# Y-Claw/Multilevel-GNN

Measured on AMD Instinct MI355X. Metric: graphs/sec fwd+bwd, 3-level GNN on 10k-node d=128 synthetic; HBM GB/s %peak, higher is better.
Workload: dtype f32; 1 GPU; configs[1]: ER graphs N=10000 E=160000 x64 per GPU, d=128, 3 GENConv(softmax, res+, LayerNorm) + projection pooling G=25000 k=2 + DiffPool 146->37->10, fp32; step = CSR build (of the next batch, on a second stream) + fwd + bwd + grad all-reduce + Adam; graphs_per_gpu=64, global_batch=64, parallelism=dp1, world_size=1, allreduce_bytes=1429768

## Files before the change

### multilevel-gnn_amd/csrc/densesage.hip

```cpp
#include "common.h"
#include "launch.h"
#include "mlgnn.h"
#include "tile_gemm.h"

namespace mlgnn {

constexpr int kDsMaxN = 160, kDsMaxC = 128, kDsMaxO = 64, kDsMaxNAdj = 48;
constexpr int kDsBlock = 1024, kDsWaves = kDsBlock / kWave;
constexpr float kDsNormEps = 1e-12f;
constexpr int kDsFwdTiles = 3;
static_assert(kDsFwdTiles * (kDsWaves / (kDsMaxO / 16)) >= kDsMaxN / 16, "row tiles of one column tile per wave");

struct DsArgs {
  const void* x; const void* adj; const void* w_rel; const void* w_root; const float* bias;
  const void* gy; const void* y; const float* rinv_in;
  void* y_out; float* rinv; void* gx; void* gadj; float* ws;
  int n; int C; int O; int adj_batched; int normalize; int ws_cols;
  int vec16;
};

template <typename AB>
__device__ __forceinline__ void ds_degrees(const AB ab, int n, int stride, float* deg, float* raw) {
  const int lane = threadIdx.x & (kWave - 1), wave = threadIdx.x / kWave;
  for (int r = wave; r < n; r += kDsWaves) {
    float s = 0.f;
    for (int j = lane; j < n; j += kWave) s += ab[(size_t)r * stride + j];
#pragma unroll
    for (int off = 32; off > 0; off >>= 1) s += __shfl_xor(s, off);
    if (lane == 0) {
      if (raw) raw[r] = s;
      deg[r] = fmaxf(s, 1.0f);
    }
  }
}

struct DsLds { int so, sx, sa, np, op; };
__host__ __device__ inline DsLds ds_lds(int n, int C, int O) {
  DsLds l;
  l.np = (n + 15) & ~15;
  l.op = (O + 15) & ~15;
  l.so = l.op + 1;
  l.sx = ((C + 31) & ~31) + 1;
  l.sa = ((n + 31) & ~31) + 1;
  return l;
}
__host__ __device__ inline int ds_fwd_floats(const DsLds& l) {
  const int first = l.np * l.sx + 2 * l.op * l.sx, then = l.np * (l.sx > l.sa ? l.sx : l.sa) + l.np * l.so;
  return first > then ? first : then;
}
inline size_t ds_fwd_lds_bytes(int n, int C, int O) {
  const DsLds l = ds_lds(n, C, O);
  return ((size_t)ds_fwd_floats(l) + l.np) * 4;
}
inline size_t ds_bwd_lds_bytes(int n, int C, int O, bool adj_grad) {
  const DsLds l = ds_lds(n, C, O);
  size_t f = (size_t)2 * l.np * l.so + 2 * l.np;
  if (adj_grad) f += (size_t)l.np * l.so + (size_t)l.np * (l.np + 1);
  return f * 4;
}

template <typename T, int V>
__device__ __forceinline__ void ds_stage_run(float* img, int stride, const T* src, int cols, int first, int count) {
  const int step = V * kDsBlock, dr = step / cols, dc = step - dr * cols;
  int e = first + V * (int)threadIdx.x;
  int r = e / cols, c = e - r * cols;
  for (int i = threadIdx.x; i < count; i += kDsBlock, e += step) {
    float v[V];
    load_t<T, V>(v, src + e);
    int rr = r, cc = c;
#pragma unroll
    for (int q = 0; q < V; ++q) {
      img[rr * stride + cc] = v[q];
      if (++cc == cols) { cc = 0; ++rr; }
    }
    c += dc; r += dr;
    if (c >= cols) { c -= cols; ++r; }
  }
}

template <typename T>
__device__ __forceinline__ void ds_stage(float* img, int stride, const T* src, int rows, int cols, int rows_p,
                                         int cols_p, int vec16) {
  constexpr int V = 16 / (int)sizeof(T);
  const int lane = threadIdx.x & (kWave - 1), wave = threadIdx.x / kWave;
  const int total = rows * cols;
  int head = total;
  if (vec16) head = min(total, (int)(((0 - reinterpret_cast<uintptr_t>(src)) & 15) / sizeof(T)));
  const int nvec = (total - head) / V;
  ds_stage_run<T, 1>(img, stride, src, cols, 0, head);
  if (nvec > 0) ds_stage_run<T, V>(img, stride, src, cols, head, nvec);
  ds_stage_run<T, 1>(img, stride, src, cols, head + V * nvec, total - head - V * nvec);
  for (int r = wave; r < rows_p; r += kDsWaves)
    for (int c = (r < rows ? cols : 0) + lane; c < cols_p; c += kWave) img[r * stride + c] = 0.f;
}

template <typename T>
__global__ __launch_bounds__(kDsBlock) void dense_sage_fwd_kernel(const DsArgs p) {
  extern __shared__ __attribute__((aligned(16))) float ds_smem[];
  const int b = blockIdx.x, tid = threadIdx.x;
  const int lane = tid & (kWave - 1), wave = tid / kWave;
  const int n = p.n, C = p.C, O = p.O;
  const DsLds L = ds_lds(n, C, O);
  const int SO = L.so, SX = L.sx, SA = L.sa;
  float* Xm_ = ds_smem;
  float* Wr_ = Xm_ + (size_t)L.np * SX;
  float* Wt_ = Wr_ + (size_t)L.op * SX;
  float* Am_ = Xm_;
  float* deg = ds_smem + ds_fwd_floats(L);
  float* Pm_ = deg - (size_t)L.np * SO;
#define P(r, c) Pm_[(r) * SO + (c)]
#define X(r, c) Xm_[(r) * SX + (c)]
#define A(r, c) Am_[(r) * SA + (c)]
  const T* xg = static_cast<const T*>(p.x) + (size_t)b * n * C;
  const T* ag = static_cast<const T*>(p.adj) + (p.adj_batched ? (size_t)b * n * n : 0);
  const int NP = (n + 15) & ~15, OP = (O + 15) & ~15;
  const int Nt = NP / 16, Ot = OP / 16;
  const int l15 = lane & 15, lq = lane >> 4;
  const int wpc = kDsWaves / Ot, j0 = (wave % Ot) * 16, first = wave / Ot;
  const bool active = first < wpc;

  ds_stage<T>(Xm_, SX, xg, n, C, NP, SX - 1, p.vec16);
  ds_stage<T>(Wr_, SX, static_cast<const T*>(p.w_rel), O, C, OP, SX - 1, p.vec16);
  ds_stage<T>(Wt_, SX, static_cast<const T*>(p.w_root), O, C, OP, SX - 1, p.vec16);
  __syncthreads();
  f32x4 keep[kDsFwdTiles];
  for_k_blocks<kDsMaxC / 32>((C + 31) >> 5, [&](auto kb) {
    constexpr int KB = decltype(kb)::value;
    float wr[8 * KB], wt[8 * KB];
    if (active) {
      frag_load<KB>(wr, [&](int k) { return Wr_[(j0 + l15) * SX + k]; });
      frag_load<KB>(wt, [&](int k) { return Wt_[(j0 + l15) * SX + k]; });
    }
    __syncthreads();
    if (active) {
#pragma unroll
      for (int s = 0; s < kDsFwdTiles; ++s) {
        const int i0 = (first + s * wpc) * 16;
        if (i0 < NP) {
          f32x4 acc;
          tile_gemm2_b_resident<KB>(wr, wt, [&](int i, int k) { return X(i0 + i, k); }, acc, keep[s]);
#pragma unroll
          for (int r = 0; r < 4; ++r) P(i0 + lq * 4 + r, j0 + l15) = acc[r];
        }
      }
    }
  });
  __syncthreads();
  ds_stage<T>(Am_, SA, ag, n, n, NP, (n + 31) & ~31, p.vec16);
  __syncthreads();
  ds_degrees(Am_, n, SA, deg, nullptr);
  f32x4 agg[kDsFwdTiles];
  if (active) {
#pragma unroll
    for (int s = 0; s < kDsFwdTiles; ++s) {
      const int i0 = (first + s * wpc) * 16;
      if (i0 < NP)
        agg[s] = tile_gemm(n,
            [&](int i, int k) { return A(i0 + i, k); },
            [&](int k, int j) { return k < n ? P(k, j0 + j) : 0.f; });
    }
  }
  __syncthreads();
  if (active) {
    const float bj = (p.bias && j0 + l15 < O) ? p.bias[j0 + l15] : 0.f;
#pragma unroll
    for (int s = 0; s < kDsFwdTiles; ++s) {
      const int i0 = (first + s * wpc) * 16;
      if (i0 < NP) {
#pragma unroll
        for (int r = 0; r < 4; ++r) {
          const int row = i0 + lq * 4 + r;
          P(row, j0 + l15) = agg[s][r] / deg[min(row, n - 1)] + keep[s][r] + bj;
        }
      }
    }
  }
  __syncthreads();
  for (int r = wave; r < n; r += kDsWaves) {
    const float v = lane < O ? P(r, lane) : 0.f;
    float ss = v * v;
#pragma unroll
    for (int off = 32; off > 0; off >>= 1) ss += __shfl_xor(ss, off);
    const float ri = p.normalize ? 1.0f / fmaxf(sqrtf(ss), kDsNormEps) : 1.0f;
    if (lane < O) stored_write<T>(p.y_out, ((size_t)b * n + r) * O + lane, v * ri);
    if (lane == 0) p.rinv[(size_t)b * n + r] = ri;
  }
}
#undef P
#undef X
#undef A

template <typename T>
__global__ __launch_bounds__(kDsBlock) void dense_sage_bwd_kernel(const DsArgs p) {
  extern __shared__ __attribute__((aligned(16))) float ds_smem[];
  const int b = blockIdx.x, tid = threadIdx.x;
  const int lane = tid & (kWave - 1), wave = tid / kWave;
  const int n = p.n, C = p.C, O = p.O;
  const DsLds L = ds_lds(n, C, O);
  const int SO = L.so, SM = L.np + 1;
  float* G_ = ds_smem;
  float* GP_ = G_ + (size_t)L.np * SO;
  float* deg = GP_ + (size_t)L.np * SO;
  float* raw = deg + L.np;
  float* Pm_ = raw + L.np;
  float* M_ = Pm_ + (size_t)L.np * SO;
#define G(r, c) G_[(r) * SO + (c)]
#define GP(r, c) GP_[(r) * SO + (c)]
#define Pm(r, c) Pm_[(r) * SO + (c)]
#define M(r, c) M_[(r) * SM + (c)]
  const StoredIn<T> xb{static_cast<const T*>(p.x) + (size_t)b * n * C};
  const StoredIn<T> ab{static_cast<const T*>(p.adj) + (p.adj_batched ? (size_t)b * n * n : 0)};
  const StoredIn<T> w_rel{static_cast<const T*>(p.w_rel)}, w_root{static_cast<const T*>(p.w_root)};
  const StoredIn<T> gyb{static_cast<const T*>(p.gy) + (size_t)b * n * O};
  const StoredIn<T> yb{static_cast<const T*>(p.y) + (size_t)b * n * O};
  const int NP = (n + 15) & ~15, OP = (O + 15) & ~15, CP = (C + 15) & ~15;
  const int Nt = NP / 16, Ot = OP / 16, Ct = CP / 16;
  const int l15 = lane & 15, lq = lane >> 4;

  ds_degrees(ab, n, n, deg, raw);
  for (int r = wave; r < NP; r += kDsWaves) {
    float gv = 0.f, yv = 0.f;
    if (r < n && lane < O) { gv = gyb[(size_t)r * O + lane]; yv = yb[(size_t)r * O + lane]; }
    float dot = gv * yv;
#pragma unroll
    for (int off = 32; off > 0; off >>= 1) dot += __shfl_xor(dot, off);
    const float ri = r < n ? p.rinv_in[(size_t)b * n + r] : 0.f;
    const float g = p.normalize ? (gv - yv * dot) * ri : gv;
    if (lane < OP) G(r, lane) = (r < n && lane < O) ? g : 0.f;
  }
  __syncthreads();
  for (int t = wave; t < Nt * Ot; t += kDsWaves) {
    const int i0 = (t / Ot) * 16, j0 = (t % Ot) * 16;
    const f32x4 acc = tile_gemm(n,
        [&](int i, int k) { return (i0 + i < n && k < n) ? ab[(size_t)k * n + i0 + i] : 0.f; },
        [&](int k, int j) { return k < n ? G(k, j0 + j) / deg[k] : 0.f; });
#pragma unroll
    for (int r = 0; r < 4; ++r) GP(i0 + lq * 4 + r, j0 + l15) = acc[r];
  }
  __syncthreads();
  const size_t gx_off = (size_t)b * n * C;
  for (int t = wave; t < Nt * Ct; t += kDsWaves) {
    const int i0 = (t / Ct) * 16, c0 = (t % Ct) * 16;
    f32x4 acc = tile_gemm(O,
        [&](int i, int k) { return k < O ? GP(i0 + i, k) : 0.f; },
        [&](int k, int j) { return (k < O && c0 + j < C) ? w_rel[(size_t)k * C + c0 + j] : 0.f; });
    const f32x4 t2 = tile_gemm(O,
        [&](int i, int k) { return k < O ? G(i0 + i, k) : 0.f; },
        [&](int k, int j) { return (k < O && c0 + j < C) ? w_root[(size_t)k * C + c0 + j] : 0.f; });
#pragma unroll
    for (int r = 0; r < 4; ++r) {
      const int row = i0 + lq * 4 + r, col = c0 + l15;
      if (row < n && col < C) stored_write<T>(p.gx, gx_off + (size_t)row * C + col, acc[r] + t2[r]);
    }
  }
  float* wsb = p.ws + (size_t)b * p.ws_cols;
  for (int t = wave; t < 2 * Ot * Ct; t += kDsWaves) {
    const int which = t / (Ot * Ct), tt = t % (Ot * Ct);
    const int o0 = (tt / Ct) * 16, c0 = (tt % Ct) * 16;
    const float* src = which == 0 ? GP_ : G_;
    const f32x4 acc = tile_gemm(n,
        [&](int i, int k) { return k < n ? src[k * SO + o0 + i] : 0.f; },
        [&](int k, int j) { return (k < n && c0 + j < C) ? xb[(size_t)k * C + c0 + j] : 0.f; });
#pragma unroll
    for (int r = 0; r < 4; ++r) {
      const int o = o0 + lq * 4 + r, c = c0 + l15;
      if (o < O && c < C) wsb[(size_t)which * O * C + (size_t)o * C + c] = acc[r];
    }
  }
  for (int o = tid; o < O; o += kDsBlock) {
    float s = 0.f;
    for (int r = 0; r < n; ++r) s += G(r, o);
    wsb[(size_t)2 * O * C + o] = s;
  }
  if (p.gadj) {
    for (int t = wave; t < Nt * Ot; t += kDsWaves) {
      const int i0 = (t / Ot) * 16, j0 = (t % Ot) * 16;
      const f32x4 acc = tile_gemm(C,
          [&](int i, int k) { return (i0 + i < n && k < C) ? xb[(size_t)(i0 + i) * C + k] : 0.f; },
          [&](int k, int j) { return (j0 + j < O && k < C) ? w_rel[(size_t)(j0 + j) * C + k] : 0.f; });
#pragma unroll
      for (int r = 0; r < 4; ++r) Pm(i0 + lq * 4 + r, j0 + l15) = acc[r];
    }
    __syncthreads();
    for (int t = wave; t < Nt * Nt; t += kDsWaves) {
      const int i0 = (t / Nt) * 16, j0 = (t % Nt) * 16;
      const f32x4 acc = tile_gemm(O,
          [&](int i, int k) { return k < O ? G(i0 + i, k) : 0.f; },
          [&](int k, int j) { return k < O ? Pm(j0 + j, k) : 0.f; });
#pragma unroll
      for (int r = 0; r < 4; ++r) M(i0 + lq * 4 + r, j0 + l15) = acc[r];
    }
    __syncthreads();
    const size_t ga_off = (size_t)b * n * n;
    for (int r = wave; r < n; r += kDsWaves) {
      float c = lane < n ? ab[(size_t)r * n + lane] * M(r, lane) : 0.f;
#pragma unroll
      for (int off = 32; off > 0; off >>= 1) c += __shfl_xor(c, off);
      const float ci = raw[r] >= 1.0f ? c / deg[r] : 0.f;
      if (lane < n) stored_write<T>(p.gadj, ga_off + (size_t)r * n + lane, (M(r, lane) - ci) / deg[r]);
    }
  }
}
#undef G
#undef GP
#undef Pm
#undef M

static bool ds_dims_ok(int64_t n, int64_t C, int64_t O) {
  return n >= 1 && n <= kDsMaxN && C >= 1 && C <= kDsMaxC && O >= 1 && O <= kDsMaxO;
}

}

using namespace mlgnn;

extern "C" int mlgnn_dense_sage_supported(int64_t n, int64_t C, int64_t O, int need_grad_adj) {
  return (ds_dims_ok(n, C, O) && (!need_grad_adj || n <= kDsMaxNAdj)) ? 1 : 0;
}

extern "C" int64_t mlgnn_dense_sage_bwd_workspace_floats(int64_t B, int64_t C, int64_t O) {
  if (B < 0 || C <= 0 || O <= 0) return MLGNN_E_SHAPE;
  return B * (2 * O * C + O);
}

extern "C" int mlgnn_dense_sage_fwd(const void* x, const void* adj, const void* w_rel, const void* w_root,
                                    const float* bias, void* y, float* rinv, int64_t B, int64_t n, int64_t C,
                                    int64_t O, int adj_batched, int normalize, int dtype, void* stream) {
  if (dtype != MLGNN_DTYPE_F32 && dtype != MLGNN_DTYPE_BF16) return MLGNN_E_DTYPE;
  if (B < 0 || !ds_dims_ok(n, C, O)) return MLGNN_E_SHAPE;
  if (B == 0) return 0;
  if (!x || !adj || !w_rel || !w_root || !y || !rinv) return MLGNN_E_NULL;
  DsArgs a = {};
  a.x = x; a.adj = adj; a.w_rel = w_rel; a.w_root = w_root;
  a.bias = bias; a.y_out = y; a.rinv = rinv;
  a.n = (int)n; a.C = (int)C; a.O = (int)O; a.adj_batched = adj_batched; a.normalize = normalize;
  a.vec16 = aligned<16>(x, adj, w_rel, w_root) ? 1 : 0;
  const size_t lds = ds_fwd_lds_bytes((int)n, (int)C, (int)O);
  static size_t fwd_attr = 0;
  if (lds > fwd_attr) {
    const int most = (int)ds_fwd_lds_bytes(kDsMaxN, kDsMaxC, kDsMaxO);
    if (const hipError_t e = allow_dynamic_lds(&dense_sage_fwd_kernel<float>, most); e != hipSuccess) return (int)e;
    if (const hipError_t e = allow_dynamic_lds(&dense_sage_fwd_kernel<bf16_t>, most); e != hipSuccess) return (int)e;
    fwd_attr = (size_t)most;
  }
  if (dtype == MLGNN_DTYPE_BF16) hipLaunchKernelGGL(dense_sage_fwd_kernel<bf16_t>, dim3((unsigned)B), dim3(kDsBlock), lds, (hipStream_t)stream, a);
  else hipLaunchKernelGGL(dense_sage_fwd_kernel<float>, dim3((unsigned)B), dim3(kDsBlock), lds, (hipStream_t)stream, a);
  return (int)hipGetLastError();
}

extern "C" int mlgnn_dense_sage_bwd(const void* grad_y, const void* y, const float* rinv, const void* x,
                                    const void* adj, const void* w_rel, const void* w_root, void* grad_x,
                                    void* grad_adj, float* grad_w, float* workspace, int64_t workspace_floats,
                                    int64_t B, int64_t n, int64_t C, int64_t O, int adj_batched, int normalize,
                                    int dtype, void* stream) {
  if (dtype != MLGNN_DTYPE_F32 && dtype != MLGNN_DTYPE_BF16) return MLGNN_E_DTYPE;
  if (B < 0 || !ds_dims_ok(n, C, O)) return MLGNN_E_SHAPE;
  if (grad_adj && n > kDsMaxNAdj) return MLGNN_E_SHAPE;
  if (!grad_w) return MLGNN_E_NULL;
  const int cols = (int)(2 * O * C + O);
  hipStream_t s = (hipStream_t)stream;
  if (B == 0) return (int)hipMemsetAsync(grad_w, 0, (size_t)cols * 4, s);
  if (!grad_y || !y || !rinv || !x || !adj || !w_rel || !w_root || !grad_x || !workspace) return MLGNN_E_NULL;
  if (workspace_floats < B * cols) return MLGNN_E_WORKSPACE;
  DsArgs a = {};
  a.x = x; a.adj = adj; a.w_rel = w_rel; a.w_root = w_root;
  a.gy = grad_y; a.y = y; a.rinv_in = rinv;
  a.gx = grad_x; a.gadj = grad_adj; a.ws = workspace; a.ws_cols = cols;
  a.n = (int)n; a.C = (int)C; a.O = (int)O; a.adj_batched = adj_batched; a.normalize = normalize;
  const size_t lds = ds_bwd_lds_bytes((int)n, (int)C, (int)O, grad_adj != nullptr);
  static size_t bwd_attr = 0;
  if (lds > bwd_attr) {
    const size_t most = ds_bwd_lds_bytes(kDsMaxN, kDsMaxC, kDsMaxO, false) > ds_bwd_lds_bytes(kDsMaxNAdj, kDsMaxC, kDsMaxO, true)
                            ? ds_bwd_lds_bytes(kDsMaxN, kDsMaxC, kDsMaxO, false) : ds_bwd_lds_bytes(kDsMaxNAdj, kDsMaxC, kDsMaxO, true);
    if (const hipError_t e = allow_dynamic_lds(&dense_sage_bwd_kernel<float>, (int)most); e != hipSuccess) return (int)e;
    if (const hipError_t e = allow_dynamic_lds(&dense_sage_bwd_kernel<bf16_t>, (int)most); e != hipSuccess) return (int)e;
    bwd_attr = most;
  }
  if (dtype == MLGNN_DTYPE_BF16) hipLaunchKernelGGL(dense_sage_bwd_kernel<bf16_t>, dim3((unsigned)B), dim3(kDsBlock), lds, s, a);
  else hipLaunchKernelGGL(dense_sage_bwd_kernel<float>, dim3((unsigned)B), dim3(kDsBlock), lds, s, a);
  int err = (int)hipGetLastError();
  if (err) return err;
  launch_reduce_partials(workspace, grad_w, (int)B, cols, s);
  return (int)hipGetLastError();
}
```

### multilevel-gnn_amd/csrc/tile_gemm.h

```cpp
#pragma once
#include "split_precision.h"
#include "dispatch.h"

namespace mlgnn {

constexpr int kTileUnroll = 8;

template <typename FA, typename FB>
__device__ __forceinline__ f32x4 tile_gemm(int kdim, FA a_at, FB b_at) {
  const int lane = threadIdx.x & (kWave - 1);
  const int l15 = lane & 15, lk = lane >> 4;
  f32x4 acc = {0.f, 0.f, 0.f, 0.f};
  for (int k0 = 0; k0 < kdim; k0 += 4 * kTileUnroll) {
    float a[kTileUnroll], b[kTileUnroll];
#pragma unroll
    for (int u = 0; u < kTileUnroll; ++u) {
      a[u] = a_at(l15, k0 + 4 * u + lk);
      b[u] = b_at(k0 + 4 * u + lk, l15);
    }
#pragma unroll
    for (int u = 0; u < kTileUnroll; ++u) acc = __builtin_amdgcn_mfma_f32_16x16x4f32(a[u], b[u], acc, 0, 0, 0);
  }
  return acc;
}

template <int KB, typename F>
__device__ __forceinline__ void frag_load(float (&f)[8 * KB], F at) {
  const int lk = (threadIdx.x & (kWave - 1)) >> 4;
#pragma unroll
  for (int u = 0; u < 8 * KB; ++u) f[u] = at(4 * u + lk);
}

template <int KB, typename FA>
__device__ __forceinline__ void tile_gemm2_b_resident(const float (&b0)[8 * KB], const float (&b1)[8 * KB], FA a_at,
                                                      f32x4& acc0, f32x4& acc1) {
  const int lane = threadIdx.x & (kWave - 1);
  const int l15 = lane & 15, lk = lane >> 4;
  acc0 = f32x4{0.f, 0.f, 0.f, 0.f};
  acc1 = f32x4{0.f, 0.f, 0.f, 0.f};
#pragma unroll
  for (int blk = 0; blk < KB; ++blk) {
    float a[kTileUnroll];
#pragma unroll
    for (int u = 0; u < kTileUnroll; ++u) a[u] = a_at(l15, 32 * blk + 4 * u + lk);
#pragma unroll
    for (int u = 0; u < kTileUnroll; ++u) {
      acc0 = __builtin_amdgcn_mfma_f32_16x16x4f32(a[u], b0[8 * blk + u], acc0, 0, 0, 0);
      acc1 = __builtin_amdgcn_mfma_f32_16x16x4f32(a[u], b1[8 * blk + u], acc1, 0, 0, 0);
    }
  }
}

template <int MAXKB, typename F>
__device__ __forceinline__ void for_k_blocks(int kb, F&& f) {
  if constexpr (MAXKB > 1) {
    if (kb < MAXKB) { for_k_blocks<MAXKB - 1>(kb, f); return; }
  }
  f(IC<MAXKB>{});
}

}
```

Measured before the change: 5557 graphs/s.

## Stage adjacency, weights and features in LDS for dense SAGE backward

The DiffPool dense SAGE backward kernel can now copy the adjacency, both weight matrices and the node features into shared memory whenever they fit and there are enough tiles to reuse them. All GEMMs then read from LDS instead of re-reading global memory per tile. Alongside that, it prefetches gy/y/rinv into registers so those loads overlap the adjacency staging, and folds the 1/deg scaling into the degree pass. It also keeps weight fragments in registers across row tiles for the gx GEMM and unrolls the bias-gradient sum. The cost is added LDS footprint near the 160 KiB limit, extra barriers, and an env var that forces either path.

```diff
diff --git a/multilevel-gnn_amd/csrc/densesage.hip b/multilevel-gnn_amd/csrc/densesage.hip
--- a/multilevel-gnn_amd/csrc/densesage.hip
+++ b/multilevel-gnn_amd/csrc/densesage.hip
@@ -1,3 +1,5 @@
+#include <cstdlib>
+
 #include "common.h"
 #include "launch.h"
 #include "mlgnn.h"
@@ -9,6 +11,9 @@
 constexpr int kDsBlock = 1024, kDsWaves = kDsBlock / kWave;
 constexpr float kDsNormEps = 1e-12f;
 constexpr int kDsFwdTiles = 3;
+constexpr int kDsRows = kDsMaxN / kDsWaves;
+static_assert(kDsRows * kDsWaves == kDsMaxN, "every padded row of g has a wave");
+constexpr int kDsGpTiles = ((kDsMaxN / 16) * (kDsMaxO / 16) + kDsWaves - 1) / kDsWaves;
 static_assert(kDsFwdTiles * (kDsWaves / (kDsMaxO / 16)) >= kDsMaxN / 16, "row tiles of one column tile per wave");
 
 struct DsArgs {
@@ -31,6 +36,19 @@
       if (raw) raw[r] = s;
       deg[r] = fmaxf(s, 1.0f);
     }
+  }
+}
+
+template <typename AB, typename F>
+__device__ __forceinline__ void ds_degrees_each(const AB ab, int n, int stride, float* deg, float* raw, F each) {
+  const int lane = threadIdx.x & (kWave - 1), wave = threadIdx.x / kWave;
+  for (int r = wave; r < n; r += kDsWaves) {
+    float s = 0.f;
+    for (int j = lane; j < n; j += kWave) s += ab[(size_t)r * stride + j];
+#pragma unroll
+    for (int off = 32; off > 0; off >>= 1) s += __shfl_xor(s, off);
+    if (lane == 0) { raw[r] = s; deg[r] = fmaxf(s, 1.0f); }
+    each(r, fmaxf(s, 1.0f));
   }
 }
 
@@ -52,11 +70,44 @@
   const DsLds l = ds_lds(n, C, O);
   return ((size_t)ds_fwd_floats(l) + l.np) * 4;
 }
-inline size_t ds_bwd_lds_bytes(int n, int C, int O, bool adj_grad) {
-  const DsLds l = ds_lds(n, C, O);
-  size_t f = (size_t)2 * l.np * l.so + 2 * l.np;
-  if (adj_grad) f += (size_t)l.np * l.so + (size_t)l.np * (l.np + 1);
-  return f * 4;
+constexpr int kDsLdsBytes = 160 * 1024;
+struct DsBwdLds { int np, so, sa, sw, base, xo, floats; };
+__host__ __device__ constexpr DsBwdLds ds_bwd_lds(int n, int C, int O, bool adj_grad, bool images) {
+  DsBwdLds l = {};
+  l.np = (n + 15) & ~15;
+  l.so = ((O + 15) & ~15) + 1;
+  l.sa = ((n + 31) & ~31) + 1;
+  l.sw = ((C + 31) & ~31) + (adj_grad ? 17 : 16);
+  l.base = 2 * l.np * l.so + 2 * l.np + (adj_grad ? l.np * l.so + l.np * (l.np + 1) : 0);
+  const int a = n * l.sa, w = 2 * O * l.sw, x = n * l.sw;
+  l.xo = adj_grad ? w : 0;
+  const int wx = adj_grad ? w + x : (w > x ? w : x);
+  l.floats = l.base + (images ? (a > wx ? a : wx) : 0);
+  return l;
+}
+constexpr size_t ds_bwd_lds_bytes(int n, int C, int O, bool adj_grad, bool images) {
+  return (size_t)ds_bwd_lds(n, C, O, adj_grad, images).floats * 4;
+}
+constexpr bool ds_bwd_images_fit(int n, int C, int O, bool adj_grad) {
+  return ds_bwd_lds_bytes(n, C, O, adj_grad, true) <= (size_t)kDsLdsBytes;
+}
+constexpr bool ds_bwd_images_pay(int n, int C, int O) {
+  const int nt = (n + 15) / 16, ct = (C + 15) / 16, ot = (O + 15) / 16;
+  return nt * ot + nt * ct + 2 * ot * ct > kDsWaves;
+}
+static_assert(ds_bwd_images_fit(146, 128, 37, false) && ds_bwd_images_fit(146, 128, 32, false), "level 1");
+static_assert(ds_bwd_images_pay(146, 128, 37) && ds_bwd_images_pay(146, 128, 32), "level 1");
+static_assert(ds_bwd_lds_bytes(146, 128, 37, false, true) == 158024, "level 1: n rows of the adjacency, not 160");
+static_assert(ds_bwd_images_fit(37, 32, 32, true) && ds_bwd_images_fit(37, 32, 10, true) &&
+              ds_bwd_images_fit(37, 32, 64, true) && ds_bwd_images_fit(10, 64, 64, true), "levels 2 and 3");
+static_assert(ds_bwd_images_pay(37, 32, 32) && ds_bwd_images_pay(37, 32, 64) && ds_bwd_images_pay(10, 64, 64) &&
+              !ds_bwd_images_pay(37, 32, 10), "levels 2 and 3: the 10-channel assignment conv keeps global operands");
+static_assert(ds_bwd_images_fit(146, 128, 48, false) && !ds_bwd_images_fit(146, 128, 49, false), "O <= 48 at n = 146");
+static_assert(ds_bwd_images_fit(kDsMaxNAdj, kDsMaxC, kDsMaxO, true), "every shape with the adjacency gradient");
+static_assert(!ds_bwd_images_fit(kDsMaxN, kDsMaxC, kDsMaxO, false), "x + g + gP alone exceed the LDS there");
+inline int ds_bwd_path_forced() {
+  static const int v = [] { const char* e = getenv("MLGNN_DS_BWD_GLOBAL"); return !e ? -1 : e[0] == '1' ? 1 : e[0] == '0' ? 0 : -1; }();
+  return v;
 }
 
 template <typename T, int V>
@@ -190,26 +241,31 @@
 #undef X
 #undef A
 
-template <typename T>
+template <typename T, bool IMG>
 __global__ __launch_bounds__(kDsBlock) void dense_sage_bwd_kernel(const DsArgs p) {
   extern __shared__ __attribute__((aligned(16))) float ds_smem[];
   const int b = blockIdx.x, tid = threadIdx.x;
   const int lane = tid & (kWave - 1), wave = tid / kWave;
   const int n = p.n, C = p.C, O = p.O;
-  const DsLds L = ds_lds(n, C, O);
-  const int SO = L.so, SM = L.np + 1;
+  const DsBwdLds L = ds_bwd_lds(n, C, O, p.gadj != nullptr, IMG);
+  const int SO = L.so, SM = L.np + 1, SA = L.sa, SW = L.sw;
   float* G_ = ds_smem;
   float* GP_ = G_ + (size_t)L.np * SO;
   float* deg = GP_ + (size_t)L.np * SO;
   float* raw = deg + L.np;
   float* Pm_ = raw + L.np;
   float* M_ = Pm_ + (size_t)L.np * SO;
+  float* Am_ = ds_smem + L.base;
+  float* Wr_ = Am_;
+  float* Wt_ = Wr_ + (size_t)O * SW;
+  float* Xm_ = Am_ + L.xo;
 #define G(r, c) G_[(r) * SO + (c)]
 #define GP(r, c) GP_[(r) * SO + (c)]
 #define Pm(r, c) Pm_[(r) * SO + (c)]
 #define M(r, c) M_[(r) * SM + (c)]
-  const StoredIn<T> xb{static_cast<const T*>(p.x) + (size_t)b * n * C};
-  const StoredIn<T> ab{static_cast<const T*>(p.adj) + (p.adj_batched ? (size_t)b * n * n : 0)};
+  const T* xg = static_cast<const T*>(p.x) + (size_t)b * n * C;
+  const T* ag = static_cast<const T*>(p.adj) + (p.adj_batched ? (size_t)b * n * n : 0);
+  const StoredIn<T> xb{xg}, ab{ag};
   const StoredIn<T> w_rel{static_cast<const T*>(p.w_rel)}, w_root{static_cast<const T*>(p.w_root)};
   const StoredIn<T> gyb{static_cast<const T*>(p.gy) + (size_t)b * n * O};
   const StoredIn<T> yb{static_cast<const T*>(p.y) + (size_t)b * n * O};
@@ -217,42 +273,95 @@
   const int Nt = NP / 16, Ot = OP / 16, Ct = CP / 16;
   const int l15 = lane & 15, lq = lane >> 4;
 
-  ds_degrees(ab, n, n, deg, raw);
-  for (int r = wave; r < NP; r += kDsWaves) {
-    float gv = 0.f, yv = 0.f;
-    if (r < n && lane < O) { gv = gyb[(size_t)r * O + lane]; yv = yb[(size_t)r * O + lane]; }
-    float dot = gv * yv;
-#pragma unroll
-    for (int off = 32; off > 0; off >>= 1) dot += __shfl_xor(dot, off);
-    const float ri = r < n ? p.rinv_in[(size_t)b * n + r] : 0.f;
-    const float g = p.normalize ? (gv - yv * dot) * ri : gv;
-    if (lane < OP) G(r, lane) = (r < n && lane < O) ? g : 0.f;
-  }
-  __syncthreads();
-  for (int t = wave; t < Nt * Ot; t += kDsWaves) {
-    const int i0 = (t / Ot) * 16, j0 = (t % Ot) * 16;
-    const f32x4 acc = tile_gemm(n,
-        [&](int i, int k) { return (i0 + i < n && k < n) ? ab[(size_t)k * n + i0 + i] : 0.f; },
-        [&](int k, int j) { return k < n ? G(k, j0 + j) / deg[k] : 0.f; });
-#pragma unroll
-    for (int r = 0; r < 4; ++r) GP(i0 + lq * 4 + r, j0 + l15) = acc[r];
-  }
-  __syncthreads();
+  float gv[kDsRows], yv[kDsRows], ri[kDsRows];
+#pragma unroll
+  for (int s = 0; s < kDsRows; ++s) {
+    const int r = wave + s * kDsWaves;
+    gv[s] = yv[s] = ri[s] = 0.f;
+    if (r < n) {
+      if (lane < O) { gv[s] = gyb[(size_t)r * O + lane]; yv[s] = yb[(size_t)r * O + lane]; }
+      ri[s] = p.rinv_in[(size_t)b * n + r];
+    }
+  }
+  if constexpr (IMG) ds_stage<T>(Am_, SA, ag, n, n, n, n, p.vec16);
+#pragma unroll
+  for (int s = 0; s < kDsRows; ++s) {
+    const int r = wave + s * kDsWaves;
+    if (r < NP) {
+      float dot = gv[s] * yv[s];
+#pragma unroll
+      for (int off = 32; off > 0; off >>= 1) dot += __shfl_xor(dot, off);
+      const float g = p.normalize ? (gv[s] - yv[s] * dot) * ri[s] : gv[s];
+      if (lane < OP) G(r, lane) = (r < n && lane < O) ? g : 0.f;
+    }
+  }
+  if constexpr (IMG) __syncthreads();
+  const auto scale_row = [&](int r, float d) { if (lane < OP) GP(r, lane) = G(r, lane) / d; };
+  if constexpr (IMG) ds_degrees_each(Am_, n, SA, deg, raw, scale_row);
+  else ds_degrees_each(ab, n, n, deg, raw, scale_row);
+  __syncthreads();
+  f32x4 gp[kDsGpTiles];
+#pragma unroll
+  for (int s = 0; s < kDsGpTiles; ++s) {
+    const int t = wave + s * kDsWaves;
+    if (t < Nt * Ot) {
+      const int i0 = (t / Ot) * 16, j0 = (t % Ot) * 16;
+      gp[s] = tile_gemm(n,
+          [&](int i, int k) {
+            if constexpr (IMG) return (i0 + i < n && k < n) ? Am_[k * SA + i0 + i] : 0.f;
+            else return (i0 + i < n && k < n) ? ab[(size_t)k * n + i0 + i] : 0.f;
+          },
+          [&](int k, int j) { return k < n ? GP(k, j0 + j) : 0.f; });
+    }
+  }
+  __syncthreads();
+#pragma unroll
+  for (int s = 0; s < kDsGpTiles; ++s) {
+    const int t = wave + s * kDsWaves;
+    if (t < Nt * Ot) {
+      const int i0 = (t / Ot) * 16, j0 = (t % Ot) * 16;
+#pragma unroll
+      for (int r = 0; r < 4; ++r) GP(i0 + lq * 4 + r, j0 + l15) = gp[s][r];
+    }
+  }
+  __syncthreads();
+  if constexpr (IMG) {
+    ds_stage<T>(Wr_, SW, w_rel.p, O, C, O, C, p.vec16);
+    ds_stage<T>(Wt_, SW, w_root.p, O, C, O, C, p.vec16);
+    __syncthreads();
+  }
   const size_t gx_off = (size_t)b * n * C;
-  for (int t = wave; t < Nt * Ct; t += kDsWaves) {
-    const int i0 = (t / Ct) * 16, c0 = (t % Ct) * 16;
-    f32x4 acc = tile_gemm(O,
-        [&](int i, int k) { return k < O ? GP(i0 + i, k) : 0.f; },
-        [&](int k, int j) { return (k < O && c0 + j < C) ? w_rel[(size_t)k * C + c0 + j] : 0.f; });
-    const f32x4 t2 = tile_gemm(O,
-        [&](int i, int k) { return k < O ? G(i0 + i, k) : 0.f; },
-        [&](int k, int j) { return (k < O && c0 + j < C) ? w_root[(size_t)k * C + c0 + j] : 0.f; });
-#pragma unroll
-    for (int r = 0; r < 4; ++r) {
-      const int row = i0 + lq * 4 + r, col = c0 + l15;
-      if (row < n && col < C) stored_write<T>(p.gx, gx_off + (size_t)row * C + col, acc[r] + t2[r]);
-    }
-  }
+  const int wpc = kDsWaves / Ct, c0 = (wave % Ct) * 16, first = wave / Ct;
+  for_k_blocks<kDsMaxO / 32>((O + 31) >> 5, [&](auto kb) {
+    constexpr int KB = decltype(kb)::value;
+    float wr[8 * KB], wt[8 * KB];
+    if (first < wpc) {
+      const bool col = c0 + l15 < C;
+      if constexpr (IMG) {
+        frag_load<KB>(wr, [&](int k) { return (k < O && col) ? Wr_[k * SW + c0 + l15] : 0.f; });
+        frag_load<KB>(wt, [&](int k) { return (k < O && col) ? Wt_[k * SW + c0 + l15] : 0.f; });
+      } else {
+        frag_load<KB>(wr, [&](int k) { return (k < O && col) ? w_rel[(size_t)k * C + c0 + l15] : 0.f; });
+        frag_load<KB>(wt, [&](int k) { return (k < O && col) ? w_root[(size_t)k * C + c0 + l15] : 0.f; });
+      }
+    }
+    if constexpr (IMG) {
+      if (L.xo == 0) __syncthreads();
+      ds_stage<T>(Xm_, SW, xg, n, C, n, C, p.vec16);
+    }
+    if (first < wpc) {
+      for (int i0 = first * 16; i0 < NP; i0 += wpc * 16) {
+        const f32x4 acc = tile_gemm_b_resident<KB>(wr, [&](int i, int k) { return k < O ? GP(i0 + i, k) : 0.f; });
+        const f32x4 t2 = tile_gemm_b_resident<KB>(wt, [&](int i, int k) { return k < O ? G(i0 + i, k) : 0.f; });
+#pragma unroll
+        for (int r = 0; r < 4; ++r) {
+          const int row = i0 + lq * 4 + r, col = c0 + l15;
+          if (row < n && col < C) stored_write<T>(p.gx, gx_off + (size_t)row * C + col, acc[r] + t2[r]);
+        }
+      }
+    }
+  });
+  if constexpr (IMG) __syncthreads();
   float* wsb = p.ws + (size_t)b * p.ws_cols;
   for (int t = wave; t < 2 * Ot * Ct; t += kDsWaves) {
     const int which = t / (Ot * Ct), tt = t % (Ot * Ct);
@@ -260,7 +369,10 @@
     const float* src = which == 0 ? GP_ : G_;
     const f32x4 acc = tile_gemm(n,
         [&](int i, int k) { return k < n ? src[k * SO + o0 + i] : 0.f; },
-        [&](int k, int j) { return (k < n && c0 + j < C) ? xb[(size_t)k * C + c0 + j] : 0.f; });
+        [&](int k, int j) {
+          if constexpr (IMG) return (k < n && c0 + j < C) ? Xm_[k * SW + c0 + j] : 0.f;
+          else return (k < n && c0 + j < C) ? xb[(size_t)k * C + c0 + j] : 0.f;
+        });
 #pragma unroll
     for (int r = 0; r < 4; ++r) {
       const int o = o0 + lq * 4 + r, c = c0 + l15;
@@ -269,15 +381,29 @@
   }
   for (int o = tid; o < O; o += kDsBlock) {
     float s = 0.f;
-    for (int r = 0; r < n; ++r) s += G(r, o);
+    int r = 0;
+    for (; r + 8 <= n; r += 8) {
+      float v[8];
+#pragma unroll
+      for (int q = 0; q < 8; ++q) v[q] = G(r + q, o);
+#pragma unroll
+      for (int q = 0; q < 8; ++q) s += v[q];
+    }
+    for (; r < n; ++r) s += G(r, o);
     wsb[(size_t)2 * O * C + o] = s;
   }
   if (p.gadj) {
     for (int t = wave; t < Nt * Ot; t += kDsWaves) {
       const int i0 = (t / Ot) * 16, j0 = (t % Ot) * 16;
       const f32x4 acc = tile_gemm(C,
-          [&](int i, int k) { return (i0 + i < n && k < C) ? xb[(size_t)(i0 + i) * C + k] : 0.f; },
-          [&](int k, int j) { return (j0 + j < O && k < C) ? w_rel[(size_t)(j0 + j) * C + k] : 0.f; });
+          [&](int i, int k) {
+            if constexpr (IMG) return (i0 + i < n && k < C) ? Xm_[(i0 + i) * SW + k] : 0.f;
+            else return (i0 + i < n && k < C) ? xb[(size_t)(i0 + i) * C + k] : 0.f;
+          },
+          [&](int k, int j) {
+            if constexpr (IMG) return (j0 + j < O && k < C) ? Wr_[(j0 + j) * SW + k] : 0.f;
+            else return (j0 + j < O && k < C) ? w_rel[(size_t)(j0 + j) * C + k] : 0.f;
+          });
 #pragma unroll
       for (int r = 0; r < 4; ++r) Pm(i0 + lq * 4 + r, j0 + l15) = acc[r];
     }
@@ -367,17 +493,30 @@
   a.gy = grad_y; a.y = y; a.rinv_in = rinv;
   a.gx = grad_x; a.gadj = grad_adj; a.ws = workspace; a.ws_cols = cols;
   a.n = (int)n; a.C = (int)C; a.O = (int)O; a.adj_batched = adj_batched; a.normalize = normalize;
-  const size_t lds = ds_bwd_lds_bytes((int)n, (int)C, (int)O, grad_adj != nullptr);
-  static size_t bwd_attr = 0;
-  if (lds > bwd_attr) {
-    const size_t most = ds_bwd_lds_bytes(kDsMaxN, kDsMaxC, kDsMaxO, false) > ds_bwd_lds_bytes(kDsMaxNAdj, kDsMaxC, kDsMaxO, true)
-                            ? ds_bwd_lds_bytes(kDsMaxN, kDsMaxC, kDsMaxO, false) : ds_bwd_lds_bytes(kDsMaxNAdj, kDsMaxC, kDsMaxO, true);
-    if (const hipError_t e = allow_dynamic_lds(&dense_sage_bwd_kernel<float>, (int)most); e != hipSuccess) return (int)e;
-    if (const hipError_t e = allow_dynamic_lds(&dense_sage_bwd_kernel<bf16_t>, (int)most); e != hipSuccess) return (int)e;
-    bwd_attr = most;
-  }
-  if (dtype == MLGNN_DTYPE_BF16) hipLaunchKernelGGL(dense_sage_bwd_kernel<bf16_t>, dim3((unsigned)B), dim3(kDsBlock), lds, s, a);
-  else hipLaunchKernelGGL(dense_sage_bwd_kernel<float>, dim3((unsigned)B), dim3(kDsBlock), lds, s, a);
+  a.vec16 = aligned<16>(x, adj, w_rel, w_root) ? 1 : 0;
+  const int forced = ds_bwd_path_forced();
+  const bool images = forced != 1 && ds_bwd_images_fit((int)n, (int)C, (int)O, grad_adj != nullptr) &&
+                      (forced == 0 || ds_bwd_images_pay((int)n, (int)C, (int)O));
+  const size_t lds = ds_bwd_lds_bytes((int)n, (int)C, (int)O, grad_adj != nullptr, images);
+  static bool bwd_attr = false;
+  if (!bwd_attr) {
+    constexpr size_t wide = ds_bwd_lds_bytes(kDsMaxN, kDsMaxC, kDsMaxO, false, false);
+    constexpr size_t adjg = ds_bwd_lds_bytes(kDsMaxNAdj, kDsMaxC, kDsMaxO, true, false);
+    constexpr int most = (int)(wide > adjg ? wide : adjg);
+    if (const hipError_t e = allow_dynamic_lds(&dense_sage_bwd_kernel<float, true>, kDsLdsBytes); e != hipSuccess) return (int)e;
+    if (const hipError_t e = allow_dynamic_lds(&dense_sage_bwd_kernel<bf16_t, true>, kDsLdsBytes); e != hipSuccess) return (int)e;
+    if (const hipError_t e = allow_dynamic_lds(&dense_sage_bwd_kernel<float, false>, most); e != hipSuccess) return (int)e;
+    if (const hipError_t e = allow_dynamic_lds(&dense_sage_bwd_kernel<bf16_t, false>, most); e != hipSuccess) return (int)e;
+    bwd_attr = true;
+  }
+  const dim3 grid((unsigned)B), block(kDsBlock);
+  if (dtype == MLGNN_DTYPE_BF16) {
+    if (images) hipLaunchKernelGGL((dense_sage_bwd_kernel<bf16_t, true>), grid, block, lds, s, a);
+    else hipLaunchKernelGGL((dense_sage_bwd_kernel<bf16_t, false>), grid, block, lds, s, a);
+  } else {
+    if (images) hipLaunchKernelGGL((dense_sage_bwd_kernel<float, true>), grid, block, lds, s, a);
+    else hipLaunchKernelGGL((dense_sage_bwd_kernel<float, false>), grid, block, lds, s, a);
+  }
   int err = (int)hipGetLastError();
   if (err) return err;
   launch_reduce_partials(workspace, grad_w, (int)B, cols, s);
diff --git a/multilevel-gnn_amd/csrc/tile_gemm.h b/multilevel-gnn_amd/csrc/tile_gemm.h
--- a/multilevel-gnn_amd/csrc/tile_gemm.h
+++ b/multilevel-gnn_amd/csrc/tile_gemm.h
@@ -51,6 +51,22 @@
   }
 }
 
+template <int KB, typename FA>
+__device__ __forceinline__ f32x4 tile_gemm_b_resident(const float (&b)[8 * KB], FA a_at) {
+  const int lane = threadIdx.x & (kWave - 1);
+  const int l15 = lane & 15, lk = lane >> 4;
+  f32x4 acc = {0.f, 0.f, 0.f, 0.f};
+#pragma unroll
+  for (int blk = 0; blk < KB; ++blk) {
+    float a[kTileUnroll];
+#pragma unroll
+    for (int u = 0; u < kTileUnroll; ++u) a[u] = a_at(l15, 32 * blk + 4 * u + lk);
+#pragma unroll
+    for (int u = 0; u < kTileUnroll; ++u) acc = __builtin_amdgcn_mfma_f32_16x16x4f32(a[u], b[8 * blk + u], acc, 0, 0, 0);
+  }
+  return acc;
+}
+
 template <int MAXKB, typename F>
 __device__ __forceinline__ void for_k_blocks(int kb, F&& f) {
   if constexpr (MAXKB > 1) {
```

Result: no change. 5587 graphs/s, median of 6 (+0.5%).
